# leejeongho3214/LightHand

Hardware: AMD Instinct MI355X
Metric: images/sec/GPU (256×256, bs=64) train+infer; EPE/AUC parity (higher is better)
Workload: dtype bf16; 1 GPU; SimpleBaseline-ResNet50 256x256 training step (fwd + JointsMSELoss + argmax decode + bwd + Adam), batch 64/GPU, 21 joints, random init (seed 9001), hipGraph replay; global_batch=64, parallelism=dp1

## Files before the change

### include/lighthand_hip.h

```cpp
#ifndef LIGHTHAND_HIP_H
#define LIGHTHAND_HIP_H

#include <stddef.h>
#include <stdint.h>

#ifdef __cplusplus
extern "C" {
#endif

typedef enum { LH_F32 = 0, LH_BF16 = 1, LH_F16 = 2 } lh_dtype;

typedef enum {
    LH_OK = 0,
    LH_ERR_ARG = -1,
    LH_ERR_HIP = -2,
    LH_ERR_UNSUPPORTED = -3
} lh_status;

int lh_version(void);
const char* lh_last_error(void);
int lh_dtype_size(int dtype);

int lh_image_to_nhwc4(const float* nchw, void* out, int n, int h, int w, int pad, int wp,
                      int dtype, void* stream);
// ... 103 lines not shown
    int out_pix_stride;
    int ntaps;
    int relu;
    signed char dh[64];
    signed char dw[64];
    int cfg[8];
} lh_igemm_desc;

int lh_igemm(const lh_igemm_desc* d, const void* in, const void* wpack, void* out,
             const void* addend, const void* addend_mask, const float* bias, const float* scale, const float* shift,
             float* stats, int dtype, void* stream);
typedef struct {
    const void* x;
    const float* mean;
    const float* invstd;
    const float* scale;
    const float* shift;
    float* partial;
    const void* mask;
    const void* x2;
    const float* mean2;
    const float* invstd2;
    float* partial2;
} lh_bn_bwd_gate;
int lh_igemm_gated_rows(const lh_igemm_desc* d, int dtype, int nterms);
int lh_igemm_gated(const lh_igemm_desc* d, const void* in, const void* wpack, void* out, const void* addend, const void* addend_mask,
                   const lh_bn_bwd_gate* gate, int dtype, void* stream);
int lh_igemm_phases_rows(const lh_igemm_desc* const* descs, int nphase, int dtype);
int lh_igemm_phases(const lh_igemm_desc* const* descs, int nphase, const void* in, const void* const* wpacks,
                    void* out, const void* addend, const void* addend_mask, const float* bias, const float* scale,
                    const float* shift, float* stats, int dtype, void* stream);
typedef struct {
    const void* w;
    size_t w_row_bytes;
    const float* bias;
    float* out;
    int n_out;
} lh_head;
int lh_igemm_phases_head(const lh_igemm_desc* const* descs, int nphase, const void* in, const void* const* wpacks,
                         const float* scale, const float* shift, const lh_head* head, int dtype, void* stream);
int lh_igemm_tile(const lh_igemm_desc* d, int dtype, int* bm, int* bp, int* ring);
int lh_igemm_config(const lh_igemm_desc* d, int dtype, int* cfg5);
int lh_igemm_candidates(const lh_igemm_desc* d, int dtype, int* cfgs, int max);
int lh_wgrad_rowfold(const lh_igemm_desc* d, int rows, const void* x, const void* dy, int dy_pix_stride,
                     int n_out, float* slab, int dtype, void* stream);
int lh_wgrad_tile(const lh_igemm_desc* d, int n_out, int n_in, int dtype, int* bo, int* bi, int* nsplit, int* ring);
// ... 211 lines not shown
```

### lighthand_amd/_lib.py

```python
import ctypes as C
import os

_HERE = os.path.dirname(os.path.abspath(__file__))
LIB_PATH = os.environ.get("LH_LIB_PATH") or os.path.join(_HERE, "liblighthand_hip.so")

LH_F32, LH_BF16, LH_F16 = 0, 1, 2
LH_FB_REDUCE_GEN, LH_FB_REDUCE_FLAT, LH_FB_REDUCE_FLAT_X, LH_FB_COEF, LH_FB_APPLY_GEN, LH_FB_APPLY_FLAT, LH_FB_APPLY_FLAT_X, LH_FB_APPLY2 = range(8)
LH_FF_GEN, LH_FF_FLAT1, LH_FF_FLAT2 = range(3)


class LightHandError(RuntimeError):
    pass


def conv_kind(depth):
    return ("staged" if depth == 0 else "pointwise" if depth == 1 else "tiled" if 2 <= depth < 10 else "dense" if 20 <= depth < 30
            else "direct" if depth == 100 else None)


class IgemmDesc(C.Structure):
    _fields_ = [("n", C.c_int), ("hi", C.c_int), ("wi", C.c_int), ("in_pix_stride", C.c_int),
                ("k_run", C.c_int), ("ho", C.c_int), ("wo", C.c_int), ("sh", C.c_int), ("sw", C.c_int),
                ("cout", C.c_int), ("OH", C.c_int), ("OW", C.c_int), ("osh", C.c_int), ("osw", C.c_int),
                ("ooh", C.c_int), ("oow", C.c_int), ("out_pix_stride", C.c_int), ("ntaps", C.c_int),
# ... 3 lines not shown
class BnFinalizeCall(C.Structure):
    _fields_ = [("stats", C.c_void_p), ("rows", C.c_int), ("count", C.c_int), ("c", C.c_int), ("gamma", C.c_void_p), ("beta", C.c_void_p),
                ("running_mean", C.c_void_p), ("running_var", C.c_void_p), ("num_batches_tracked", C.c_void_p), ("momentum", C.c_float),
                ("eps", C.c_float), ("scale", C.c_void_p), ("shift", C.c_void_p), ("save_mean", C.c_void_p), ("save_invstd", C.c_void_p)]


class FuseDesc(C.Structure):
    _fields_ = [("x", C.c_void_p * 4), ("scale", C.c_void_p * 4), ("shift", C.c_void_p * 4),
                ("log2up", C.c_int * 4), ("nterms", C.c_int), ("relu", C.c_int), ("relu_mask", C.c_void_p),
                ("fin", C.POINTER(BnFinalizeCall) * 4), ("l2_touch", C.c_void_p), ("l2_touch_bytes", C.c_size_t)]


class FuseBwdDesc(C.Structure):
    _fields_ = [("dout", C.c_void_p), ("out", C.c_void_p), ("x", C.c_void_p * 4), ("scale", C.c_void_p * 4),
                ("shift", C.c_void_p * 4), ("save_mean", C.c_void_p * 4), ("save_invstd", C.c_void_p * 4), ("dx", C.c_void_p * 4),
                ("dgamma", C.c_void_p * 4), ("dbeta", C.c_void_p * 4), ("log2up", C.c_int * 4),
                ("accumulate", C.c_int * 4), ("nterms", C.c_int), ("relu", C.c_int),
                ("relu_mask", C.c_void_p), ("strips_cap", C.c_int), ("pre_partial", C.c_void_p), ("pre_rows", C.c_int),
                ("l2_touch", C.c_void_p), ("l2_touch_bytes", C.c_size_t), ("pre_partial2", C.c_void_p)]


class BnBwdGate(C.Structure):
    _fields_ = [("x", C.c_void_p), ("mean", C.c_void_p), ("invstd", C.c_void_p), ("scale", C.c_void_p), ("shift", C.c_void_p),
                ("partial", C.c_void_p), ("mask", C.c_void_p), ("x2", C.c_void_p), ("mean2", C.c_void_p), ("invstd2", C.c_void_p), ("partial2", C.c_void_p)]


class IgemmCall(C.Structure):
    _fields_ = [("d", C.POINTER(IgemmDesc)), ("in_", C.c_void_p), ("wpack", C.c_void_p), ("out", C.c_void_p), ("addend", C.c_void_p),
                ("addend_mask", C.c_void_p), ("bias", C.c_void_p), ("scale", C.c_void_p), ("shift", C.c_void_p), ("stats", C.c_void_p)]


class WgradCall(C.Structure):
    _fields_ = [("d", C.POINTER(IgemmDesc)), ("rows", C.c_int), ("x", C.c_void_p), ("dy", C.c_void_p), ("dy_pix_stride", C.c_int),
                ("n_out", C.c_int), ("n_in", C.c_int), ("workspace", C.c_void_p), ("grad", C.c_void_p), ("so", C.c_long), ("si", C.c_long),
                ("sr", C.c_long), ("ss", C.c_long), ("taps_rs", C.POINTER(C.c_int)), ("accumulate", C.c_int)]


class WgradTableInfo(C.Structure):
    _fields_ = [("bo", C.c_int), ("bi", C.c_int), ("kps", C.c_int), ("depth", C.c_int), ("n_problems", C.c_int), ("n_fold", C.c_int),
                ("n_items", C.c_int), ("n_fold_items", C.c_int), ("fold_lds", C.c_int), ("target_stages", C.c_int), ("nsplit_max", C.c_int),
                ("run_parts", C.c_int), ("off_items", C.c_size_t), ("off_fold_args", C.c_size_t), ("off_fold_items", C.c_size_t),
                ("table_bytes", C.c_size_t), ("workspace_bytes", C.c_size_t)]


class FuseFwdCall(C.Structure):
    _fields_ = [("d", C.POINTER(FuseDesc)), ("out", C.c_void_p), ("n", C.c_int), ("h", C.c_int), ("w", C.c_int), ("c", C.c_int)]

# ... 191 lines not shown
```

### lighthand_amd/bn_gate.py

```python
import ctypes as C

import torch

from . import _lib
from .graph import _Call, _ptr


class BnGate:
    def _note_gate(self, out, terms, bn_state, relu_bits):
        if not (self.training and self.with_bwd) or any(l != 0 for _, _, l in terms):
            return
        bn_terms = [i for i, (_, bn, _) in enumerate(terms) if bn is not None]
        if relu_bits is None:
            if len(terms) == 1 and bn_terms:
                self._gate_info[id(out)] = dict(raw=terms[0][0], st=bn_state[0])
        elif len(terms) == 2 and all(a.c == out.c for a, _, _ in terms):
            if len(bn_terms) == 1:
                self._gate_info[id(out)] = dict(raw=terms[bn_terms[0]][0], st=bn_state[bn_terms[0]], mask=relu_bits)
            elif len(bn_terms) == 2:
                self._gate_info[id(out)] = dict(raw=terms[0][0], st=bn_state[0], mask=relu_bits, raw2=terms[1][0], st2=bn_state[1])

    def _gate_kind(self, gi, x, masked_addend):
        if gi is None or x.c != x.c_valid:
            return None
        uses = len(self._uses.get(id(x), []))
        if gi.get("mask") is not None:
            ok = self.opt.bn_gate_tail and (uses == 1 or (uses == 2 and masked_addend))
            return None if not ok else "mask2" if gi.get("raw2") is not None else "mask"
        return "x" if uses == 1 else None

    def _cfg_gateable(self, cfg, kind, nbytes):
        kernel = _lib.conv_kind(cfg[2])
        pw, tiled = kernel in ("pointwise", "direct"), kernel in ("tiled", "dense")
        opt, mb = self.opt, nbytes / (1 << 20)
        if not (tiled or (pw and opt.bn_gate_pw)):
            return False
        if kind == "mask2":
            return kernel == "pointwise" and opt.bn_gate_tail2 and mb <= opt.bn_gate_tail_max_mb
        if kind == "mask":
            return mb <= (opt.bn_gate_tail_max_mb if pw else min(opt.bn_gate_tail_max_mb, opt.bn_gate_tiled_tail_max_mb))
        return mb <= (opt.bn_gate_pw_max_mb if pw else opt.bn_gate_max_mb)

    def _make_gate(self, gi, partial, partial2=None):
        st = gi["st"]
        gate = _lib.BnBwdGate(gi["raw"].buf.data_ptr(), st["mean"].data_ptr(), st["invstd"].data_ptr(), st["scale"].data_ptr(),
                              st["shift"].data_ptr(), partial.data_ptr(), _ptr(gi.get("mask")))
        if partial2 is not None:
            st2 = gi["st2"]
            gate.x2, gate.mean2, gate.invstd2, gate.partial2 = gi["raw2"].buf.data_ptr(), st2["mean"].data_ptr(), st2["invstd"].data_ptr(), partial2.data_ptr()
        self.keep.append(gate)
        return gate

    def _gated_dgrad(self, dd, dy, pk, x, dx, addend, amask, gi, gkind, what):
        two = gkind == "mask2"
        rows = self.lib.lh_igemm_gated_rows(C.byref(dd), self.dt, 2 if two else 1)
        partial = self._alloc(rows * 2 * x.c, dtype=torch.float32)
        partial2 = self._alloc(rows * 2 * x.c, dtype=torch.float32) if two else None
        gate = self._make_gate(gi, partial, partial2)
        self.keep.append(dd)
        c = _Call(self.lib.lh_igemm_gated, (C.byref(dd), _ptr(dy), _ptr(pk), _ptr(dx), _ptr(addend), _ptr(amask), C.byref(gate), self.dt),
                  what + " + BN-backward gate" + (" (mask bits)" if gi.get("mask") is not None else ""))
        c.keep = dd
        c.ig = dict(src=1, dst=3, addend=4, addend_mask=5)
        self.bwd.append(c)
        self._gated[id(x)] = (partial, rows, partial2)

    def _gate_meta(self, dd, x):
        c = self.bwd[-1]
        if getattr(c, "fn", None) is not self.lib.lh_igemm_gated:
            return None, 0.0
        g = self._gated[id(x)]
        terms = 2 if len(g) > 2 and g[2] is not None else 1
        name = self._kname(dd, stats=True)
        if name.startswith("igemm_pw_kernel"):
            name = name[:-1] + f", {terms}>"
        elif name.startswith("conv3x3_direct_kernel"):
            name = name[:-1] + ", true>"
        elif name.startswith("igemm_ring_kernel"):
            name = name.replace("igemm_ring_kernel", "igemm_ring_gated_kernel", 1)
        return name, float(terms) * x.pixels * x.c * self.es + (x.pixels * x.c / 8 if "mask" in c.what else 0.0)
```

### lighthand_amd/csrc/igemm.hip

```cpp
#include "common.h"
#include <algorithm>

#include "igemm_args.h"
#include "multi.h"

static int prepare(const lh_igemm_call& q, int dtype, bool has_head, IgemmArgs* out, ConvPlan* plan) {
    const lh_igemm_desc* d = q.d;
    LH_REQUIRE(d && q.in && q.wpack && (q.out || has_head), "lh_igemm: null pointer");
    const int es = lh_dtype_size(dtype);
    LH_REQUIRE(es > 0, "lh_igemm: bad dtype %d", dtype);
    const int epc = 16 / es;
    LH_REQUIRE(d->ntaps >= 0 && d->ntaps <= 64, "lh_igemm: ntaps %d out of range", d->ntaps);
    LH_REQUIRE(d->k_run > 0 && d->k_run % epc == 0, "lh_igemm: k_run %d must be a multiple of %d", d->k_run, epc);
    LH_REQUIRE(d->cout > 0 && d->cout % epc == 0, "lh_igemm: cout %d must be a multiple of %d", d->cout, epc);
    LH_REQUIRE(d->out_pix_stride % epc == 0 && d->out_pix_stride >= d->cout, "lh_igemm: bad out_pix_stride %d", d->out_pix_stride);
    LH_REQUIRE(d->in_pix_stride > 0 && (d->in_pix_stride * es) % 4 == 0, "lh_igemm: bad in_pix_stride");
    LH_REQUIRE(d->n > 0 && d->ho > 0 && d->wo > 0 && d->hi > 0 && d->wi > 0, "lh_igemm: bad sizes");
    LH_REQUIRE((d->ho - 1) * d->osh + d->ooh < d->OH && (d->wo - 1) * d->osw + d->oow < d->OW && d->ooh >= 0 && d->oow >= 0,
               "lh_igemm: output placement exceeds the %dx%d image", d->OH, d->OW);
    LH_REQUIRE(!q.addend_mask || (q.addend && d->out_pix_stride == d->cout), "lh_igemm: addend_mask needs an addend and a dense output (mask bits index 16-byte chunks)");
    LH_REQUIRE((q.scale == nullptr) == (q.shift == nullptr), "lh_igemm: scale and shift must come together");
    if (int rc = lh_conv_plan(d, dtype, plan)) return rc;

    IgemmArgs a = {};
// ... 14 lines not shown
    *out = a;
    return LH_OK;
}

static int attach_gate(IgemmArgs& a, const lh_igemm_desc* d, const lh_bn_bwd_gate* gate, const ConvPlan& p, int dtype) {
    LH_REQUIRE(gate->x && gate->mean && gate->invstd && gate->partial && (gate->mask || (gate->scale && gate->shift)),
               "lh_igemm_gated: null pointer in the gate (the sign of the activation comes from scale + shift or from mask)");
    LH_REQUIRE(!a.bias && !a.scale && !d->relu && a.nphase == 1 && !a.head_w, "lh_igemm_gated: a data gradient carries no bias / affine / ReLU / phases");
    LH_REQUIRE(!gate->mask || d->out_pix_stride == d->cout, "lh_igemm_gated: gate.mask needs a dense output (mask bits index 16-byte chunks)");
    a.gx = (const unsigned char*)gate->x; a.gmean = gate->mean; a.ginv = gate->invstd; a.gscale = gate->scale; a.gshift = gate->shift;
    a.gmask = (const unsigned char*)gate->mask;
    a.stats = gate->partial;
    if (gate->x2) {
        LH_REQUIRE(gate->mask && gate->mean2 && gate->invstd2 && gate->partial2, "lh_igemm_gated: a second BatchNorm term (x2) needs mask, mean2, invstd2, partial2");
        a.gx2 = (const unsigned char*)gate->x2; a.gmean2 = gate->mean2; a.ginv2 = gate->invstd2; a.stats2 = gate->partial2;
    }
    if (!(lh_kind_gated(p.kind) && lh_dtype_size(dtype) == 2)) {
        lh_set_error("lh_igemm_gated: the launch runs neither on a tiled LDS-DMA configuration nor on a persistent kernel (ring depth %d)", p.cfg.depth);
        return LH_ERR_UNSUPPORTED;
    }
    if (gate->x2 && !lh_kind_gates_two(p.kind)) {
        lh_set_error("lh_igemm_gated: two BatchNorm terms are gated by the pointwise kernel only (ring depth %d)", p.cfg.depth);
        return LH_ERR_UNSUPPORTED;
    }
    return LH_OK;
}

static int attach_phases(IgemmArgs& a, const ConvPlan& p, const lh_igemm_desc* const* descs, const void* const* wpacks, int nphase) {
    LH_REQUIRE(!lh_kind_persistent(p.kind), "lh_igemm_phases: the persistent kernels take single launches only");
    LH_REQUIRE(p.kind != LH_CONV_STAGED, "lh_igemm_phases: the form is not supported by the LDS-DMA kernel");
    a.nphase = nphase;
    a.phase_blocks = ceil_div(a.M, p.cfg.bp) * ceil_div(a.cout, p.cfg.bm);
    for (int i = 0; i < nphase; ++i) {
        const lh_igemm_desc* q = descs[i];
        a.ph_w[i] = (const unsigned char*)wpacks[i];
        a.ph_ntaps[i] = q->ntaps; a.ph_tw[i] = 1; a.ph_dh0[i] = a.ph_dhs[i] = a.ph_dw0[i] = a.ph_dws[i] = 0;
        if (q->ntaps > 0)
            LH_REQUIRE(lh_tap_grid(q, &a.ph_tw[i], &a.ph_dh0[i], &a.ph_dhs[i], &a.ph_dw0[i], &a.ph_dws[i]) && a.ph_w[i],
                       "lh_igemm_phases: phase %d has an irregular tap list or no weights", i);
        a.ph_ooh[i] = q->ooh; a.ph_oow[i] = q->oow;
        a.ph_row0[i] = i * ceil_div(a.M, p.cfg.bp);
    }
    return LH_OK;
}

static int attach_head(IgemmArgs& a, const ConvPlan& p, const lh_head* head, int es) {
// ... 97 lines not shown
```

### lighthand_amd/csrc/igemm_args.h

```cpp
#pragma once
#include "common.h"
#include "igemm_ring_cfgs.h"

struct IgemmArgs {
    const unsigned char* in;
    const unsigned char* w;
    unsigned char* out;
    const unsigned char* addend;
    const unsigned char* addend_mask;
    const unsigned char* zero;
    unsigned char* dump;
    const float* bias;
    const float* scale;
    const float* shift;
    float* stats;
    const unsigned char* gx;
    const float* gmean;
    const float* ginv;
    const float* gscale;
    const float* gshift;
    const unsigned char* gmask;
    const unsigned char* gx2;
    const float* gmean2;
    const float* ginv2;
    float* stats2;
    const unsigned char* head_w;
    const float* head_bias;
    float* head_out;
    int head_j, head_wstride;
    int n, hi, wi, in_pix_stride, k_run, kspt, kpad;
    int ho, wo, M, sh, sw, cout;
    int OH, OW, osh, osw, ooh, oow, out_pix_stride;
    int ntaps, relu;
    int nphase, phase_blocks;
    const unsigned char* ph_w[4];
    int ph_ntaps[4], ph_tw[4], ph_dh0[4], ph_dhs[4], ph_dw0[4], ph_dws[4], ph_ooh[4], ph_oow[4], ph_row0[4];
    int xcd;
    int pw_g, pw_cb;
    int tw, dh0, dhs, dw0, dws;
    signed char dh[64];
    signed char dw[64];
};

struct RingCfg {
    int bm, bp, depth, kb;
};

enum LhConvKind { LH_CONV_NONE, LH_CONV_STAGED, LH_CONV_POINTWISE, LH_CONV_TILED, LH_CONV_DENSE, LH_CONV_DIRECT };
enum { LH_POINTWISE_DEPTH = 1, LH_DIRECT_DEPTH = 100 };

static inline LhConvKind lh_conv_kind(int depth) {
    return depth == 0 ? LH_CONV_STAGED : depth == LH_POINTWISE_DEPTH ? LH_CONV_POINTWISE : depth >= 2 && depth < 10 ? LH_CONV_TILED
         : depth >= LH_DENSE_DEPTH && depth < LH_DENSE_DEPTH + 10 ? LH_CONV_DENSE : depth == LH_DIRECT_DEPTH ? LH_CONV_DIRECT : LH_CONV_NONE;
}
static inline int lh_ring_depth(const RingCfg& c) { return lh_conv_kind(c.depth) == LH_CONV_DENSE ? c.depth - LH_DENSE_DEPTH : c.depth; }
static inline bool lh_kind_persistent(LhConvKind k) { return k == LH_CONV_POINTWISE || k == LH_CONV_DIRECT; }
static inline bool lh_kind_gated(LhConvKind k) { return k != LH_CONV_STAGED && k != LH_CONV_NONE; }
static inline bool lh_kind_gates_two(LhConvKind k) { return k == LH_CONV_POINTWISE; }

struct ConvPlan {
    LhConvKind kind;
    RingCfg cfg;
};

static inline int lh_pw_lds_bytes(int bm, int kc, int pt, int gate = 0) {
// ... 27 lines not shown
```

### lighthand_amd/csrc/igemm_wave_epilogue.h

```cpp
#pragma once
#include "common.h"
#include "igemm_args.h"

#ifndef LH_ABL
#define LH_ABL 0
#endif

template <typename T, int BM, int PT, bool STATS, int GATE = 0, typename PixFn, int NS, int NS3>
__device__ __forceinline__ void wave_epilogue(const IgemmArgs& p, f32x4 (&acc)[BM / 16][PT], unsigned char* stg, const float* cst,
                                              const int cblk, const int lane, PixFn&& pix, float (&s1)[NS][8], float (&s2)[NS][8],
                                              float (&s3)[NS3][8]) {
    constexpr int ES = sizeof(T), EPC = 8, SUBW = 64, NSB = BM / SUBW, RS = SUBW * ES + 8;
    const int q = lane >> 4, pl = lane & 15;
    const int rrow = lane >> 3, rch = lane & 7;
#pragma unroll
    for (int sb = 0; sb < NSB; ++sb) {
        __builtin_amdgcn_sched_barrier(0);
#pragma unroll
        for (int it = 0; it < 4; ++it) {
            const int i = sb * 4 + it;
            const int col = i * 16 + q * 4;
            const float4 sv = GATE ? float4{1.f, 1.f, 1.f, 1.f} : *reinterpret_cast<const float4*>(cst + col);
            const float4 bv = GATE ? float4{0.f, 0.f, 0.f, 0.f} : *reinterpret_cast<const float4*>(cst + BM + col);
#pragma unroll
// ... 26 lines not shown
                    c = *reinterpret_cast<const float4*>(cst + 2 * BM + cc + 4 * h);
                    d = *reinterpret_cast<const float4*>(cst + 3 * BM + cc + 4 * h);
                }
                gmean[4 * h] = a.x; gmean[4 * h + 1] = a.y; gmean[4 * h + 2] = a.z; gmean[4 * h + 3] = a.w;
                ginv[4 * h] = b.x; ginv[4 * h + 1] = b.y; ginv[4 * h + 2] = b.z; ginv[4 * h + 3] = b.w;
                if constexpr (GATE != 2) {
                    gsc[4 * h] = c.x; gsc[4 * h + 1] = c.y; gsc[4 * h + 2] = c.z; gsc[4 * h + 3] = c.w;
                    gsh[4 * h] = d.x; gsh[4 * h + 1] = d.y; gsh[4 * h + 2] = d.z; gsh[4 * h + 3] = d.w;
                }
                if constexpr (GATE == 2) {
                    const float4 a2 = *reinterpret_cast<const float4*>(cst + 4 * BM + cc + 4 * h), b2 = *reinterpret_cast<const float4*>(cst + 5 * BM + cc + 4 * h);
                    gmean2[4 * h] = a2.x; gmean2[4 * h + 1] = a2.y; gmean2[4 * h + 2] = a2.z; gmean2[4 * h + 3] = a2.w;
                    ginv2[4 * h] = b2.x; ginv2[4 * h + 1] = b2.y; ginv2[4 * h + 2] = b2.z; ginv2[4 * h + 3] = b2.w;
                }
            }
        }
#pragma unroll
        for (int k = 0; k < NP; ++k) {
            opix[k] = col_ok ? pix(k * 8 + rrow) : -1L;
            ad[k] = uint4{0u, 0u, 0u, 0u};
            mb[k] = 0xffu;
            if (p.addend) {
                const long eoff = opix[k] * p.out_pix_stride + col0;
                ad[k] = *reinterpret_cast<const uint4*>(opix[k] >= 0 ? p.addend + eoff * ES : p.zero);
                if (p.addend_mask) mb[k] = *(opix[k] >= 0 ? p.addend_mask + eoff / EPC : p.zero);
            }
            if constexpr (GATE) {
                const long eoff = opix[k] * p.out_pix_stride + col0;
                xd[k] = *reinterpret_cast<const uint4*>(opix[k] >= 0 ? p.gx + eoff * ES : p.zero);
                gm[k] = 0xffu;
                if (p.gmask) gm[k] = *(opix[k] >= 0 ? p.gmask + eoff / EPC : p.zero);
                if constexpr (GATE == 2) xd2[k] = *reinterpret_cast<const uint4*>(opix[k] >= 0 ? p.gx2 + eoff * ES : p.zero);
            }
        }
#pragma unroll
        for (int k = 0; k < NP; ++k) {
            const int row = k * 8 + rrow;
            const unsigned char* src = stg + row * RS + rch * 16;
            const uint2 lo = *reinterpret_cast<const uint2*>(src);
            const uint2 hi = *reinterpret_cast<const uint2*>(src + 8);
            uint4 u = uint4{lo.x, lo.y, hi.x, hi.y};
            if (p.addend || p.relu) {
                float v[EPC];
                unpack16<T>(u, v);
                if (p.addend) {
                    float av[EPC];
                    unpack16<T>(ad[k], av);
// ... 79 lines not shown
```

### lighthand_amd/engine.py

```python
import ctypes as C

import torch

from . import _lib
from ._lib import FuseBwdDesc, FuseDesc, IgemmDesc, check, conv_kind
from .batch_groups import BatchGroups
from .bn_gate import BnGate
from .graph import BN_EPS, BN_MOMENTUM, PRECISIONS, Act, GraphBuilder, _Call, _Marker, _desc, _ptr, _taps_array
from .infer_rewrites import InferRewrites
from .options import PlanOptions
from .runner import Runner
from .tuner import Tuner
from .weight_packs import WeightPacks
from .wgrad_schedule import WgradSchedule


class Plan(Tuner, WgradSchedule, BatchGroups, InferRewrites, WeightPacks, BnGate, Runner):

    def __init__(self, model, n, h, w, precision="fp32", training=True, backward=None, device=None, wgrad_bucket_bytes=None, options=None):
        self.lib = _lib.load()
        self.opt = options if options is not None else PlanOptions.from_env()
        self.precision = precision
        self.tdtype = PRECISIONS[precision]
        self.dt = _lib.dtype_code(self.tdtype)
# ... 103 lines not shown

    def _dgrad(self, descs, dy, packs, x, what):
        dx = self._act_grad(x)
        first = self._first_write(x)
        if not first and len(descs) > 1:
            keep = [i for i, dd in enumerate(descs) if dd.ntaps > 0]
            descs, packs = [descs[i] for i in keep], [packs[i] for i in keep]
        addend, amask = (None if first else dx), None
        pend = self._masked_addend.pop(id(x), None)
        if pend is not None:
            assert first
            addend, amask = pend
        kind = "masked" if amask is not None else ("plain" if addend is not None else None)
        if self._phase_rows(descs) > 0:
            self._tune(descs, addend=kind)
            self._igemm_phases(self.bwd, descs, dy, packs, dx, addend, None, None, what, addend_mask=amask)
            yield max(descs, key=lambda d: d.ntaps), sum(d.ntaps for d in descs)
            return
        for dd, pk in zip(descs, packs):
            in_branch = self._emit_group > 1 or self._cur_lane != 0 or self._in_branch
            gi = self._gate_info.get(id(x)) if (self.opt.bn_gate and first and len(descs) == 1 and self.es == 2 and
                                                (self.n_lanes == 1 or (self.opt.bn_gate_branches and not in_branch))) else None
            gkind, gbytes = self._gate_kind(gi, x, amask is not None), x.pixels * x.c * self.es
            self._tune([dd], addend=kind, role="dgrad", gate=(gkind, gbytes) if gkind else None)
            cfg = (C.c_int * 5)()
            if gkind and self.lib.lh_igemm_config(C.byref(dd), self.dt, cfg) == 0 and self._cfg_gateable(cfg, gkind, gbytes):
                self._gated_dgrad(dd, dy, pk, x, dx, addend, amask, gi, gkind, what)
            else:
                self._igemm(self.bwd, dd, dy, pk, dx, addend, None, None, what, addend_mask=amask)
            yield dd, dd.ntaps

    def _patch(self, call, relu=None, **ptrs):
        a = list(call.args)
        ig = call.ig or self._IG
        for k, v in ptrs.items():
            a[ig[k]] = v
        call.args = tuple(a)
        if relu is not None:
            for d in (call.keep if isinstance(call.keep, list) else [call.keep]):
                d.relu = int(relu)

    _IGP = dict(src=2, dst=4, addend=5, addend_mask=6, bias=7, scale=8, shift=9, stats=10)

    def _phase_rows(self, descs):
        if len(descs) < 2 or len(descs) > 4:
            return -1
        arr = (C.POINTER(IgemmDesc) * len(descs))(*[C.pointer(d) for d in descs])
        return self.lib.lh_igemm_phases_rows(arr, len(descs), self.dt)

    def _igemm_phases(self, lst, descs, src, packs, dst, addend, bias, stats, what, produces=None, addend_mask=None):
        arr = (C.POINTER(IgemmDesc) * len(descs))(*[C.pointer(d) for d in descs])
# ... 77 lines not shown
        y.stats_rows = rows
        return y.stats

    def _stats_for(self, y, descs):
        rows = [self.lib.lh_igemm_stats_rows(C.byref(d), self.dt) for d in descs]
        self._alloc_stats(y, sum(rows))
        offs, o = [], 0
        for r in rows:
            offs.append(o)
            o += r * 2 * y.c * 4
        return offs

    def _compile(self):
        consumers_bn = set()
        for kind, nd in self.nodes:
            if kind == "fuse":
                for a, bn, _ in nd["terms"]:
                    if bn is not None:
                        consumers_bn.add(id(a))
        self._bn_inputs = consumers_bn
        self._nwrites = {}
        self._masked_addend = {}
        self._gate_info, self._gated = {}, {}
        self._bnrelu_info = {}
        self._uses = {}
        for kind, nd in self.nodes:
            if kind in ("conv", "deconv", "maxpool"):
                self._uses.setdefault(id(nd["x"]), []).append((kind, nd))
            elif kind == "fuse":
                for a, _, _ in nd["terms"]:
                    self._uses.setdefault(id(a), []).append((kind, nd))
            elif kind == "output":
                self._uses.setdefault(id(nd["y"]), []).append((kind, nd))
        items = self._batch_order()
        bwd_blocks, group_forced = {}, {}
        for item in items:
            gid = None
            if len(item) > 1:
                self._n_groups += 1
                gid = self._n_groups
                self._forced = self._tune_group([self.nodes[i][1] for i in item]) if self.nodes[item[0]][0] == "conv" else None
                group_forced[item[0]] = self._forced
            for j, i in enumerate(item):
                (kind, nd), lane = self.nodes[i], self.node_lanes[i]
                if self._forced is not None:
                    self._forced["member"] = j
# ... 184 lines not shown
        if not self.with_bwd:
            return
        rs_arr = _taps_array(all_rs)
        gw = self.grads[nd["w"] + ".weight"]
        pad_out = y.c != cout
        gtmp = self._alloc(y.c, cin, k, k, dtype=torch.float32) if pad_out else gw

        def tune_launch(xp, dyp, ws, grad, sp):
            check(self.lib.lh_wgrad_fused(C.byref(d), 0, xp, dyp, y.c, y.c, cin, ws, grad, cin * k * k, k * k, k, 1, rs_arr, 0, self.dt, sp),
                  "autotune lh_wgrad_fused")
        self._tune_wgrad(d, y.c, cin, y.c, tune_launch, y.c * cin * k * k)
        slab_bytes = self.lib.lh_wgrad_workspace_bytes(C.byref(d), y.c, cin, self.dt)
        self._ws_wgrad = max(self._ws_wgrad, slab_bytes)
        dpacks, ddescs = [], []
        if x.needs_grad:
            for ph in range(s):
                for pw in range(s):
                    sub = [(r, q) for r, q in all_rs if (ph + p - r) % s == 0 and (pw + p - q) % s == 0]
                    tp = [((ph + p - r) // s, (pw + p - q) // s) for r, q in sub]
                    gh, gw_ = (x.h - ph + s - 1) // s, (x.w - pw + s - 1) // s
                    dd = _desc(y.n, y.h, y.w, y.c, y.c if pad_out else cout, gh, gw_, 1, 1, x.c, x.h, x.w, s, s, ph, pw, x.c, tp)
                    ddescs.append(dd)
                    dpacks.append(self._pack(wt, cin, cout, (k * k, cin * k * k, k, 1), sub, nd["w"] + " dgrad pack"))

        def emit():
            dy = self._act_grad(y)
            a = [C.byref(d), 0, xbuf.data_ptr(), dy.data_ptr(), y.c, y.c, cin, 0, gtmp.data_ptr(), cin * k * k, k * k, k, 1, rs_arr, 0, self.dt]
            wl = self._wgrad_call(a, nd["w"] + " wgrad", slab_bytes, flops, (x.pixels * x.c + y.pixels * y.c) * self.es, wbufs=(xbuf, dy), keep_desc=d)
            if pad_out:
                wl.append(self._copy4(gw, gtmp[:cout].view_as(gw), "head grad crop", lane=1))
            if nd["bias"]:
                gb_ = self.grads[nd["bias"]]
                if y is self.out_act:
                    dn = self.dout_nchw
                    ws = self._alloc(self.lib.lh_channel_sum_workspace_bytes(dn.shape[1]), dtype=torch.uint8)
                    wl.append(_Call(self.lib.lh_channel_sum_nchw, (dn.data_ptr(), dn.shape[0], dn.shape[1], dn.shape[2] * dn.shape[3],
                                                                          gb_.data_ptr(), ws.data_ptr()), "head bias grad"))
                else:
                    wl.append(self._bias_grad(dy, y, cout, gb_))
            if x.needs_grad:
                for dd, ntaps in self._dgrad(ddescs, dy, dpacks, x, nd["w"] + " dgrad"):
                    batched = ntaps != dd.ntaps or (len(ddescs) > 1 and self.bwd[-1].ig is not None)
                    gname, gbytes = self._gate_meta(dd, x)
                    self.profile_meta.append(("bwd", self.bwd[-1], gname or self._kname(dd), 2.0 * dd.n * dd.ho * dd.wo * cin * cout * ntaps,
                                              gbytes + ((x.pixels * x.c + y.pixels * y.c) * self.es if batched else
                                                        (dd.n * dd.ho * dd.wo * x.c + y.pixels * y.c / (s * s)) * self.es)))
        blk.append(emit)

    def _c_stem(self, nd, blk, bias):
        x, y, k, s, p = nd["x"], nd["y"], nd["k"], nd["s"], nd["p"]
        wt = self.params[nd["w"] + ".weight"]
        cout = wt.shape[0]
        kr = (k * 4 + 7) // 8 * 8
        hp, wp = x.h + 2 * p, x.w + 2 * p + 2
        assert (y.w - 1) * s * 4 + kr <= wp * 4
        self.img_nchw = self._alloc(x.n, 3, x.h, x.w, dtype=torch.float32)
        img = self._alloc(x.n, hp, wp, 4)
        self.img_nhwc4, self.img_pad, self.img_wp = img, p, wp
        self.fwd.append(_Call(self.lib.lh_image_to_nhwc4, (self.img_nchw.data_ptr(), img.data_ptr(), x.n, x.h, x.w, p, wp, self.dt), "image transform"))
        self._image_call_index = len(self.fwd) - 1
        self._mirror_call = _Call(self.lib.lh_nhwc4_mirror, (img.data_ptr(), x.n, x.h, x.w, p, wp, self.dt), "image mirror")
        stage = self._alloc(cout, k, kr // 4, 4, dtype=torch.float32, zero=True)
        self.packs.append(self._copy4(stage[:, :, :k, :3], wt.detach().permute(0, 2, 3, 1), "stem weight staging"))
# ... 373 lines not shown
```

### lighthand_amd/options.py

```python
import dataclasses
import os
from dataclasses import dataclass


def _on(v):
    return v != "0"


def _int_tuple(v):
    return tuple(int(t) for t in v.split(",")) if v else None


def _l2_touch(v):
    return {"0": 0, "2": 2}.get(v, 1)


def _sw(env, default, parse=_on):
    return dataclasses.field(default=default, metadata={"env": env, "parse": parse})


@dataclass(frozen=True)
class PlanOptions:
    autotune: bool = _sw("LH_AUTOTUNE", True)
    tune_cold: bool = _sw("LH_TUNE_COLD", True)
    tune_iters: int = _sw("LH_TUNE_ITERS", 4, lambda v: max(1, int(v)))
# ... 6 lines not shown
    wgrad_table_stragglers: bool = _sw("LH_WGRAD_TABLE_STRAGGLERS", True)
    wgrad_table_force: tuple = _sw("LH_WGRAD_TABLE_FORCE", None, _int_tuple)
    wgrad_table_tune_min: int = _sw("LH_WGRAD_TABLE_TUNE_MIN", 20000, int)
    wgrad_group: int = _sw("LH_WGRAD_GROUP", None, int)
    wgrad_lanes: int = _sw("LH_WGRAD_LANES", None, int)
    bn_gate: bool = _sw("LH_BN_GATE", True)
    bn_gate_pw: bool = _sw("LH_BN_GATE_PW", True)
    bn_gate_tail: bool = _sw("LH_BN_GATE_TAIL", True)
    bn_gate_tail2: bool = _sw("LH_BN_GATE_TAIL2", True)
    bn_gate_branches: bool = _sw("LH_BN_GATE_BRANCHES", True)
    bn_gate_max_mb: float = _sw("LH_BN_GATE_MAX_MB", 9.0, float)
    bn_gate_pw_max_mb: float = _sw("LH_BN_GATE_PW_MAX_MB", 1024.0, float)
    bn_gate_tail_max_mb: float = _sw("LH_BN_GATE_TAIL_MAX_MB", 1024.0, float)
    bn_gate_tiled_tail_max_mb: float = _sw("LH_BN_GATE_TILED_TAIL_MAX_MB", 1024.0, float)
    late_pack: bool = _sw("LH_LATE_PACK", True)
    tail_spread: bool = _sw("LH_TAIL_SPREAD", True)
    stem_direct: bool = _sw("LH_STEM_DIRECT", True)
    bn_pool: bool = _sw("LH_BN_POOL", True)
    pool_gate: bool = _sw("LH_POOL_GATE", True)
    fuse_bottleneck: bool = _sw("LH_FUSE_BOTTLENECK", True)
    l2_touch: int = _sw("LH_L2_TOUCH", 1, _l2_touch)
    l2_touch_max_mb: float = _sw("LH_L2_TOUCH_MAX_MB", 3.0, float)

    @classmethod
    def from_env(cls, environ=os.environ):
        return cls(**{f.name: f.metadata["parse"](environ[f.metadata["env"]]) for f in dataclasses.fields(cls) if f.metadata["env"] in environ})

    def replace(self, **kw):
        return dataclasses.replace(self, **kw)
```

### lighthand_amd/tuner.py

```python
import ctypes as C
import os

import torch

from . import _lib
from ._lib import FuseBwdDesc, FuseDesc, IgemmDesc, check
from .graph import Act, _Call, _Marker, _desc, _ptr, _taps_array


def _record_time(key, choice, ms):
    path = os.environ.get("LH_TUNE_TIMES")
    if path:
        with open(path, "a") as f:
            f.write(repr((key, tuple(choice), float(ms))) + "\n")


class Tuner:
    _TUNE_CACHE = {}

    force_cfg = None

    force_wgrad = None

    _tune_file_loaded = False
# ... 134 lines not shown
            else:
                stream = torch.cuda.current_stream()
                a, b = torch.cuda.Event(enable_timing=True), torch.cuda.Event(enable_timing=True)
                a.record(stream)
                for _ in range(iters):
                    go()
                b.record(stream)
                b.synchronize()
                t = a.elapsed_time(b)
            if surcharge is not None:
                t += surcharge(cand) * iters
            _record_time(key, cand, t)
            if self.opt.tune_log if log is None else log:
                print(f"[tune {note(cand) if callable(note) else note}] {cand}: {t / iters * 1e3:7.1f} us", flush=True)
            if best is None or t < best[0]:
                best = (t, cand)
        return best[1]

    def _remember(self, key, choice):
        type(self)._TUNE_CACHE[key] = choice
        type(self)._tune_measured.add(key)
        return choice

    def _tune(self, descs, with_stats=False, addend=None, role=None, gate=None):
        if not self.opt.autotune:
            return
        if self._forced is not None and role in self._forced and len(descs) == 1:
            descs[0].cfg[0], descs[0].cfg[1], descs[0].cfg[2], descs[0].cfg[3] = self._forced[role]
            return
        lead = max(descs, key=lambda d: d.ntaps)
        if lead.ntaps == 0:
            return
        key = (self.dt, with_stats) + tuple(self._desc_key(d) for d in descs) + ((addend,) if addend else ()) + (("gate-" + gate[0],) if gate else ())
        hit = type(self)._TUNE_CACHE.get(key) if type(self).force_cfg is None else None
        buf, n = self._igemm_candidates(lead)
        cands = [tuple(buf[5 * i:5 * i + 4]) for i in range(n)]
        if len(descs) > 1:
            cands = [c for c in cands if c[2] not in (1, 100)]
        if len(descs) > 1 and self._phase_rows(descs) <= 0:
            cands = []
        if hit is not None and hit != (0, 0, 0, 0) and hit not in cands:
            hit = None
        if hit is None:
            if type(self).force_cfg is not None:
                forced = type(self).force_cfg(cands) if cands else None
                for d in descs:
                    d.cfg[0], d.cfg[1], d.cfg[2], d.cfg[3] = forced or (0, 0, 0, 0)
                return
            hit = (0, 0, 0, 0)
            if len(cands) > 1:
                es = self.es
                kpad = (lead.k_run * es + 127) // 128 * 128
                src = self._scratch("in", lead.n * lead.hi * lead.wi * lead.in_pix_stride * es + 256)
                dst = self._scratch("out", lead.n * lead.OH * lead.OW * lead.out_pix_stride * es + 256)
                packs = [self._scratch(f"pack{i}", (d.cout + 255) // 256 * 256 * max(d.ntaps, 1) * kpad + 256) for i, d in enumerate(descs)]
                rows = max((lead.n * lead.ho * lead.wo + 63) // 64, 1024) * len(descs)
                stats = self._scratch("stats", rows * 2 * lead.cout * 4 + 256) if with_stats else None
                dense = lead.out_pix_stride == lead.cout
                add = self._scratch("addend", lead.n * lead.OH * lead.OW * lead.out_pix_stride * es + 256) if addend else None
                amask = self._scratch("amask", lead.n * lead.OH * lead.OW * lead.out_pix_stride * es // 16 + 256) if addend == "masked" and dense else None
                sp = torch.cuda.current_stream().cuda_stream
                if len(descs) > 1:
                    arr = (C.POINTER(IgemmDesc) * len(descs))(*[C.pointer(d) for d in descs])
                    parr = (C.c_void_p * len(descs))(*[pk.data_ptr() for pk in packs])

                    def run():
                        check(self.lib.lh_igemm_phases(arr, len(descs), src.data_ptr(), parr, dst.data_ptr(), _ptr(add), _ptr(amask), None, None, None,
                                                       _ptr(stats), self.dt, sp), "autotune lh_igemm_phases")
                else:
                    def run():
                        check(self.lib.lh_igemm(C.byref(lead), src.data_ptr(), packs[0].data_ptr(), dst.data_ptr(), _ptr(add), _ptr(amask), None, None, None,
                                                _ptr(stats), self.dt, sp), "autotune lh_igemm")
                run_gated, penalty = None, 0.0
                if gate is not None and len(descs) == 1:
                    nout = lead.n * lead.OH * lead.OW * lead.out_pix_stride
                    gx = self._scratch("gate_x", nout * es + 256)
                    gvec = self._scratch("gate_vec", 4 * lead.cout * 4 + 256).view(torch.float32)
                    gvec[:4 * lead.cout] = 1.0
                    gpart = self._scratch("stats", rows * 2 * lead.cout * 4 + 256)
                    gbits = self._scratch("gate_bits", nout * es // 16 + 256) if gate[0] != "x" else None
                    c_ = lead.cout
                    gt = _lib.BnBwdGate(gx.data_ptr(), gvec.data_ptr(), gvec.data_ptr() + 4 * c_, gvec.data_ptr() + 8 * c_, gvec.data_ptr() + 12 * c_,
                                        gpart.data_ptr(), _ptr(gbits))
                    if gate[0] == "mask2":
                        gt.x2, gt.mean2, gt.invstd2 = self._scratch("gate_x2", nout * es + 256).data_ptr(), gvec.data_ptr(), gvec.data_ptr() + 4 * c_
                        gt.partial2 = self._scratch("gate_part2", rows * 2 * lead.cout * 4 + 256).data_ptr()

                    def run_gated():
                        check(self.lib.lh_igemm_gated(C.byref(lead), src.data_ptr(), packs[0].data_ptr(), dst.data_ptr(), _ptr(add), _ptr(amask),
                                                      C.byref(gt), self.dt, sp), "autotune lh_igemm_gated")
                    penalty = (4.0 if gate[0] == "mask2" else 2.0) * gate[1] / 4.5e12 * 1e3 + 2e-3

                def gated(cfg):
                    return run_gated is not None and self._cfg_gateable(cfg, gate[0], gate[1])

                def apply(cfg):
                    for d in descs:
                        d.cfg[0], d.cfg[1], d.cfg[2], d.cfg[3] = cfg
                    return run_gated if gated(cfg) else None
                shape = f"{role or ''} {lead.k_run}x{lead.ntaps}->{lead.cout} M={lead.n * lead.ho * lead.wo} addend={addend} gate={gate and gate[0]}"
                hit = self._fastest(key, cands, apply, run, [src[:lead.n * lead.hi * lead.wi * lead.in_pix_stride * es]], cold=self.opt.tune_cold,
                                    note=lambda cfg: shape + ("" if run_gated is None else "+" if gated(cfg) else "-"),
                                    surcharge=None if run_gated is None else lambda cfg: 0.0 if gated(cfg) else penalty)
            self._remember(key, hit)
        for d in descs:
            d.cfg[0], d.cfg[1], d.cfg[2], d.cfg[3] = hit

    def _tune_wgrad(self, d, n_out, n_in, dy_stride, launch, grad_floats, tag=()):
        if not self.opt.autotune:
# ... 185 lines not shown
```

Measured before the change: 7640 images/s.

## Compute stride-2 downsample dgrad compactly and fuse it as subsampled addend into gated dgrad

At ResNet stage boundaries, the 1x1 stride-2 downsample conv's input gradient is now computed as a compact ceil(H/2) x ceil(W/2) tensor. It is read as a subsampled addend inside the sibling 1x1 stride-1 gated dgrad epilogue, which also carries the BN-backward mask gate. This avoids writing and reading a full-resolution, mostly zero scattered dgrad and lets the boundary activation qualify for the BN gate. In exchange it adds magic-division index math in the epilogue, a new tuner key variant and a pointwise-kernel-only restriction, with a fallback to the old path when the gated config is not eligible.

```diff
diff --git a/include/lighthand_hip.h b/include/lighthand_hip.h
--- a/include/lighthand_hip.h
+++ b/include/lighthand_hip.h
@@ -149,6 +149,9 @@
     const float* mean2;
     const float* invstd2;
     float* partial2;
+    int addend_sub;
+    int addend_h;
+    int addend_w;
 } lh_bn_bwd_gate;
 int lh_igemm_gated_rows(const lh_igemm_desc* d, int dtype, int nterms);
 int lh_igemm_gated(const lh_igemm_desc* d, const void* in, const void* wpack, void* out, const void* addend, const void* addend_mask,
diff --git a/lighthand_amd/_lib.py b/lighthand_amd/_lib.py
--- a/lighthand_amd/_lib.py
+++ b/lighthand_amd/_lib.py
@@ -49,7 +49,8 @@
 
 class BnBwdGate(C.Structure):
     _fields_ = [("x", C.c_void_p), ("mean", C.c_void_p), ("invstd", C.c_void_p), ("scale", C.c_void_p), ("shift", C.c_void_p),
-                ("partial", C.c_void_p), ("mask", C.c_void_p), ("x2", C.c_void_p), ("mean2", C.c_void_p), ("invstd2", C.c_void_p), ("partial2", C.c_void_p)]
+                ("partial", C.c_void_p), ("mask", C.c_void_p), ("x2", C.c_void_p), ("mean2", C.c_void_p), ("invstd2", C.c_void_p), ("partial2", C.c_void_p),
+                ("addend_sub", C.c_int), ("addend_h", C.c_int), ("addend_w", C.c_int)]
 
 
 class IgemmCall(C.Structure):
diff --git a/lighthand_amd/bn_gate.py b/lighthand_amd/bn_gate.py
--- a/lighthand_amd/bn_gate.py
+++ b/lighthand_amd/bn_gate.py
@@ -25,9 +25,32 @@
             return None
         uses = len(self._uses.get(id(x), []))
         if gi.get("mask") is not None:
+            if uses == 2 and not masked_addend and gi.get("raw2") is None and self._boundary_rec(x) is not None:
+                return "mask-sub"
             ok = self.opt.bn_gate_tail and (uses == 1 or (uses == 2 and masked_addend))
             return None if not ok else "mask2" if gi.get("raw2") is not None else "mask"
         return "x" if uses == 1 else None
+
+    def _boundary_rec(self, x):
+        opt = self.opt
+        rec = self._ds_dgrad.get(id(x))
+        if rec is None or rec["taken"] or not (opt.bn_gate_boundary and opt.bn_gate_tail and opt.bn_gate_pw) or self.n_lanes != 1:
+            return None
+        uses = self._uses.get(id(x), [])
+        forms = sorted((kind, nd["k"], nd["s"], nd["p"]) if kind == "conv" else (kind,) for kind, nd in uses)
+        if forms != [("conv", 1, 1, 0), ("conv", 1, 2, 0)] or not any(nd is rec["nd"] for _, nd in uses):
+            return None
+        return rec
+
+    def _boundary_dgrad(self, x):
+        rec = self._ds_dgrad[id(x)]
+        rec["taken"] = True
+        dd, y = rec["desc"], rec["y"]
+        t = self._alloc(x.n, rec["th"], rec["tw"], x.c)
+        self._tune([dd], role="dgrad", tag="compact")
+        self._igemm(self.bwd, dd, self._act_grad(y), rec["pack"], t, None, None, None, rec["nd"]["w"] + " dgrad (compact, the next launch's subsampled addend)")
+        self.profile_meta.append(("bwd", self.bwd[-1], self._kname(dd), rec["flops"], (x.n * rec["th"] * rec["tw"] * x.c + y.pixels * y.c) * self.es))
+        return t
 
     def _cfg_gateable(self, cfg, kind, nbytes):
         kernel = _lib.conv_kind(cfg[2])
@@ -37,6 +60,8 @@
             return False
         if kind == "mask2":
             return kernel == "pointwise" and opt.bn_gate_tail2 and mb <= opt.bn_gate_tail_max_mb
+        if kind == "mask-sub":
+            return kernel == "pointwise" and mb <= opt.bn_gate_tail_max_mb
         if kind == "mask":
             return mb <= (opt.bn_gate_tail_max_mb if pw else min(opt.bn_gate_tail_max_mb, opt.bn_gate_tiled_tail_max_mb))
         return mb <= (opt.bn_gate_pw_max_mb if pw else opt.bn_gate_max_mb)
@@ -57,9 +82,12 @@
         partial = self._alloc(rows * 2 * x.c, dtype=torch.float32)
         partial2 = self._alloc(rows * 2 * x.c, dtype=torch.float32) if two else None
         gate = self._make_gate(gi, partial, partial2)
+        sub = gkind == "mask-sub"
+        if sub:
+            gate.addend_sub, gate.addend_h, gate.addend_w = 1, addend.shape[1], addend.shape[2]
         self.keep.append(dd)
         c = _Call(self.lib.lh_igemm_gated, (C.byref(dd), _ptr(dy), _ptr(pk), _ptr(dx), _ptr(addend), _ptr(amask), C.byref(gate), self.dt),
-                  what + " + BN-backward gate" + (" (mask bits)" if gi.get("mask") is not None else ""))
+                  what + " + BN-backward gate" + (" (mask bits, subsampled addend)" if sub else " (mask bits)" if gi.get("mask") is not None else ""))
         c.keep = dd
         c.ig = dict(src=1, dst=3, addend=4, addend_mask=5)
         self.bwd.append(c)
@@ -78,4 +106,6 @@
             name = name[:-1] + ", true>"
         elif name.startswith("igemm_ring_kernel"):
             name = name.replace("igemm_ring_kernel", "igemm_ring_gated_kernel", 1)
-        return name, float(terms) * x.pixels * x.c * self.es + (x.pixels * x.c / 8 if "mask" in c.what else 0.0)
+        compact = c.args[4] and "subsampled addend" in c.what
+        return name, (float(terms) * x.pixels * x.c * self.es + (x.pixels * x.c / 8 if "mask" in c.what else 0.0)
+                      + (x.n * ((x.h + 1) // 2) * ((x.w + 1) // 2) * x.c * self.es if compact else 0.0))
diff --git a/lighthand_amd/csrc/igemm.hip b/lighthand_amd/csrc/igemm.hip
--- a/lighthand_amd/csrc/igemm.hip
+++ b/lighthand_amd/csrc/igemm.hip
@@ -60,6 +60,20 @@
     if (gate->x2 && !lh_kind_gates_two(p.kind)) {
         lh_set_error("lh_igemm_gated: two BatchNorm terms are gated by the pointwise kernel only (ring depth %d)", p.cfg.depth);
         return LH_ERR_UNSUPPORTED;
+    }
+    if (gate->addend_sub) {
+        LH_REQUIRE(gate->addend_sub == 1 && a.addend && !a.addend_mask && !gate->x2,
+                   "lh_igemm_gated: a subsampled addend is subsampled by two, needs an addend and goes with neither addend_mask nor x2");
+        LH_REQUIRE(d->ho == d->OH && d->wo == d->OW && d->osh == 1 && d->osw == 1 && d->ooh == 0 && d->oow == 0 &&
+                   gate->addend_h == (d->ho + 1) / 2 && gate->addend_w == (d->wo + 1) / 2,
+                   "lh_igemm_gated: a subsampled addend needs a dense output placement and a compact size of ceil(%d / 2) x ceil(%d / 2)", d->ho, d->wo);
+        if (p.kind != LH_CONV_POINTWISE) {
+            lh_set_error("lh_igemm_gated: a subsampled addend is read by the pointwise kernel only (ring depth %d)", p.cfg.depth);
+            return LH_ERR_UNSUPPORTED;
+        }
+        a.add_sub = 1; a.add_h = gate->addend_h; a.add_w = gate->addend_w;
+        lh_div_magic((unsigned)(d->ho * d->wo), &a.add_mhw, &a.add_shw);
+        lh_div_magic((unsigned)d->wo, &a.add_mw, &a.add_sw);
     }
     return LH_OK;
 }
diff --git a/lighthand_amd/csrc/igemm_args.h b/lighthand_amd/csrc/igemm_args.h
--- a/lighthand_amd/csrc/igemm_args.h
+++ b/lighthand_amd/csrc/igemm_args.h
@@ -40,7 +40,16 @@
     int tw, dh0, dhs, dw0, dws;
     signed char dh[64];
     signed char dw[64];
+    int add_sub, add_h, add_w;
+    unsigned add_mhw, add_shw, add_mw, add_sw;
 };
+
+static inline void lh_div_magic(unsigned d, unsigned* magic, unsigned* shift) {
+    unsigned l = 0;
+    while ((1ul << l) < d) ++l;
+    *shift = 31 + l;
+    *magic = (unsigned)(((1ul << (31 + l)) + d - 1) / d);
+}
 
 struct RingCfg {
     int bm, bp, depth, kb;
diff --git a/lighthand_amd/csrc/igemm_wave_epilogue.h b/lighthand_amd/csrc/igemm_wave_epilogue.h
--- a/lighthand_amd/csrc/igemm_wave_epilogue.h
+++ b/lighthand_amd/csrc/igemm_wave_epilogue.h
@@ -72,7 +72,17 @@
             mb[k] = 0xffu;
             if (p.addend) {
                 const long eoff = opix[k] * p.out_pix_stride + col0;
-                ad[k] = *reinterpret_cast<const uint4*>(opix[k] >= 0 ? p.addend + eoff * ES : p.zero);
+                const unsigned char* asrc = opix[k] >= 0 ? p.addend + eoff * ES : p.zero;
+                if constexpr (GATE == 1) {
+                    if (p.add_sub) {
+                        const unsigned m = (unsigned)opix[k];
+                        const unsigned n = (unsigned)(((unsigned long)m * p.add_mhw) >> p.add_shw), rem = m - n * (unsigned)(p.ho * p.wo);
+                        const unsigned y = (unsigned)(((unsigned long)rem * p.add_mw) >> p.add_sw), x = rem - y * (unsigned)p.wo;
+                        const long apix = (int)((n * p.add_h + (y >> 1)) * p.add_w + (x >> 1));
+                        asrc = (opix[k] >= 0 && !((y | x) & 1u)) ? p.addend + (apix * p.out_pix_stride + col0) * ES : p.zero;
+                    }
+                }
+                ad[k] = *reinterpret_cast<const uint4*>(asrc);
                 if (p.addend_mask) mb[k] = *(opix[k] >= 0 ? p.addend_mask + eoff / EPC : p.zero);
             }
             if constexpr (GATE) {
diff --git a/lighthand_amd/engine.py b/lighthand_amd/engine.py
--- a/lighthand_amd/engine.py
+++ b/lighthand_amd/engine.py
@@ -149,11 +149,17 @@
             gi = self._gate_info.get(id(x)) if (self.opt.bn_gate and first and len(descs) == 1 and self.es == 2 and
                                                 (self.n_lanes == 1 or (self.opt.bn_gate_branches and not in_branch))) else None
             gkind, gbytes = self._gate_kind(gi, x, amask is not None), x.pixels * x.c * self.es
+            if gkind == "mask-sub":
+                kind = "sub"
             self._tune([dd], addend=kind, role="dgrad", gate=(gkind, gbytes) if gkind else None)
             cfg = (C.c_int * 5)()
             if gkind and self.lib.lh_igemm_config(C.byref(dd), self.dt, cfg) == 0 and self._cfg_gateable(cfg, gkind, gbytes):
+                if gkind == "mask-sub":
+                    addend = self._boundary_dgrad(x)
                 self._gated_dgrad(dd, dy, pk, x, dx, addend, amask, gi, gkind, what)
             else:
+                if gkind == "mask-sub":
+                    self._tune([dd], addend=None, role="dgrad")
                 self._igemm(self.bwd, dd, dy, pk, dx, addend, None, None, what, addend_mask=amask)
             yield dd, dd.ntaps
 
@@ -277,6 +283,7 @@
         self._nwrites = {}
         self._masked_addend = {}
         self._gate_info, self._gated = {}, {}
+        self._ds_dgrad = {}
         self._bnrelu_info = {}
         self._uses = {}
         for kind, nd in self.nodes:
@@ -507,6 +514,12 @@
                     dd = _desc(y.n, y.h, y.w, y.c, y.c if pad_out else cout, gh, gw_, 1, 1, x.c, x.h, x.w, s, s, ph, pw, x.c, tp)
                     ddescs.append(dd)
                     dpacks.append(self._pack(wt, cin, cout, (k * k, cin * k * k, k, 1), sub, nd["w"] + " dgrad pack"))
+        ds_rec = None
+        if x.needs_grad and (k, s, p) == (1, 2, 0):
+            th, tw = (x.h + 1) // 2, (x.w + 1) // 2
+            ds_rec = self._ds_dgrad[id(x)] = dict(
+                nd=nd, y=y, pack=dpacks[0], th=th, tw=tw, taken=False, flops=2.0 * y.n * th * tw * cin * cout,
+                desc=_desc(y.n, y.h, y.w, y.c, y.c if pad_out else cout, th, tw, 1, 1, x.c, th, tw, 1, 1, 0, 0, x.c, [(0, 0)]))
 
         def emit():
             dy = self._act_grad(y)
@@ -523,7 +536,7 @@
                                                                           gb_.data_ptr(), ws.data_ptr()), "head bias grad"))
                 else:
                     wl.append(self._bias_grad(dy, y, cout, gb_))
-            if x.needs_grad:
+            if x.needs_grad and not (ds_rec and ds_rec["taken"]):
                 for dd, ntaps in self._dgrad(ddescs, dy, dpacks, x, nd["w"] + " dgrad"):
                     batched = ntaps != dd.ntaps or (len(ddescs) > 1 and self.bwd[-1].ig is not None)
                     gname, gbytes = self._gate_meta(dd, x)
diff --git a/lighthand_amd/options.py b/lighthand_amd/options.py
--- a/lighthand_amd/options.py
+++ b/lighthand_amd/options.py
@@ -1,6 +1,6 @@
 import dataclasses
 import os
-from dataclasses import dataclass
+from dataclasses import InitVar, dataclass
 
 
 def _on(v):
@@ -53,9 +53,28 @@
     l2_touch: int = _sw("LH_L2_TOUCH", 1, _l2_touch)
     l2_touch_max_mb: float = _sw("LH_L2_TOUCH_MAX_MB", 3.0, float)
 
+    bn_gate_boundary: InitVar[bool] = True
+    BOUNDARY_ENV = "LH_BN_GATE_BOUNDARY"
+
+    def __post_init__(self, bn_gate_boundary):
+        object.__setattr__(self, "bn_gate_boundary", bool(bn_gate_boundary))
+
+    def _value(self):
+        return tuple(getattr(self, f.name) for f in dataclasses.fields(self)) + (self.bn_gate_boundary,)
+
+    def __eq__(self, other):
+        return other.__class__ is self.__class__ and self._value() == other._value()
+
+    def __hash__(self):
+        return hash(self._value())
+
     @classmethod
     def from_env(cls, environ=os.environ):
-        return cls(**{f.name: f.metadata["parse"](environ[f.metadata["env"]]) for f in dataclasses.fields(cls) if f.metadata["env"] in environ})
+        kw = {f.name: f.metadata["parse"](environ[f.metadata["env"]]) for f in dataclasses.fields(cls) if f.metadata["env"] in environ}
+        if cls.BOUNDARY_ENV in environ:
+            kw["bn_gate_boundary"] = _on(environ[cls.BOUNDARY_ENV])
+        return cls(**kw)
 
     def replace(self, **kw):
+        kw.setdefault("bn_gate_boundary", self.bn_gate_boundary)
         return dataclasses.replace(self, **kw)
diff --git a/lighthand_amd/tuner.py b/lighthand_amd/tuner.py
--- a/lighthand_amd/tuner.py
+++ b/lighthand_amd/tuner.py
@@ -180,7 +180,7 @@
         type(self)._tune_measured.add(key)
         return choice
 
-    def _tune(self, descs, with_stats=False, addend=None, role=None, gate=None):
+    def _tune(self, descs, with_stats=False, addend=None, role=None, gate=None, tag=None):
         if not self.opt.autotune:
             return
         if self._forced is not None and role in self._forced and len(descs) == 1:
@@ -189,7 +189,8 @@
         lead = max(descs, key=lambda d: d.ntaps)
         if lead.ntaps == 0:
             return
-        key = (self.dt, with_stats) + tuple(self._desc_key(d) for d in descs) + ((addend,) if addend else ()) + (("gate-" + gate[0],) if gate else ())
+        key = (self.dt, with_stats) + tuple(self._desc_key(d) for d in descs) + ((addend,) if addend else ()) + (("gate-" + gate[0],) if gate else ()) \
+            + ((tag,) if tag else ())
         hit = type(self)._TUNE_CACHE.get(key) if type(self).force_cfg is None else None
         buf, n = self._igemm_candidates(lead)
         cands = [tuple(buf[5 * i:5 * i + 4]) for i in range(n)]
@@ -218,6 +219,7 @@
                 add = self._scratch("addend", lead.n * lead.OH * lead.OW * lead.out_pix_stride * es + 256) if addend else None
                 amask = self._scratch("amask", lead.n * lead.OH * lead.OW * lead.out_pix_stride * es // 16 + 256) if addend == "masked" and dense else None
                 sp = torch.cuda.current_stream().cuda_stream
+                add_plain = None if addend == "sub" else add
                 if len(descs) > 1:
                     arr = (C.POINTER(IgemmDesc) * len(descs))(*[C.pointer(d) for d in descs])
                     parr = (C.c_void_p * len(descs))(*[pk.data_ptr() for pk in packs])
@@ -227,7 +229,7 @@
                                                        _ptr(stats), self.dt, sp), "autotune lh_igemm_phases")
                 else:
                     def run():
-                        check(self.lib.lh_igemm(C.byref(lead), src.data_ptr(), packs[0].data_ptr(), dst.data_ptr(), _ptr(add), _ptr(amask), None, None, None,
+                        check(self.lib.lh_igemm(C.byref(lead), src.data_ptr(), packs[0].data_ptr(), dst.data_ptr(), _ptr(add_plain), _ptr(amask), None, None, None,
                                                 _ptr(stats), self.dt, sp), "autotune lh_igemm")
                 run_gated, penalty = None, 0.0
                 if gate is not None and len(descs) == 1:
@@ -243,6 +245,8 @@
                     if gate[0] == "mask2":
                         gt.x2, gt.mean2, gt.invstd2 = self._scratch("gate_x2", nout * es + 256).data_ptr(), gvec.data_ptr(), gvec.data_ptr() + 4 * c_
                         gt.partial2 = self._scratch("gate_part2", rows * 2 * lead.cout * 4 + 256).data_ptr()
+                    if gate[0] == "mask-sub":
+                        gt.addend_sub, gt.addend_h, gt.addend_w = 1, (lead.ho + 1) // 2, (lead.wo + 1) // 2
 
                     def run_gated():
                         check(self.lib.lh_igemm_gated(C.byref(lead), src.data_ptr(), packs[0].data_ptr(), dst.data_ptr(), _ptr(add), _ptr(amask),
```

Result: no change. 7680 images/s (median of 6 runs) (+0.5%).
